# skipperro/selkies-gstreamer

Measured on AMD Instinct MI355X. Metric: encoded fps + glass-to-glass p50 ms at 1920x1080; concurrent 60fps sessions/node, higher is better.
Workload: dtype uint8 pixels / int32 integer transforms (bit-exact vs CPU reference); 1 GPU; model=H.264 Constrained Baseline CAVLC, striped stripes 64px, CRF 25, global_batch=8, seq_len=1, parallelism=session-parallel dp1 x 8 sessions/GPU, resolution=1920x1080, backend=hip, deblock=auto, me_full=True, upload_overlap=False, frames_in_flight=1, num_refs=1, numa_node_rank0=0

## Files before the change

csrc/kernels/h264_kernels.hip:

```cpp
#include "h264_gpu.h"
#include "../codec/color.h"
#include "../codec/h264_mb.h"
#include "../codec/h264_ep.h"

namespace sk {
namespace h264 {
namespace gpu {

__device__ __forceinline__ int lane_id() { return threadIdx.x & 63; }

__device__ __forceinline__ void wave_sync() {
    __builtin_amdgcn_fence(__ATOMIC_RELEASE, "wavefront");
    __builtin_amdgcn_wave_barrier();
    __builtin_amdgcn_fence(__ATOMIC_ACQUIRE, "wavefront");
}

__device__ __forceinline__ int wave_sum(int v) {
    v += __builtin_amdgcn_mov_dpp(v, 0xB1, 0xF, 0xF, false);
    v += __builtin_amdgcn_mov_dpp(v, 0x4E, 0xF, 0xF, false);
    v += __builtin_amdgcn_mov_dpp(v, 0x124, 0xF, 0xF, false);
    v += __builtin_amdgcn_mov_dpp(v, 0x128, 0xF, 0xF, false);
    return __builtin_amdgcn_readlane(v, 0) + __builtin_amdgcn_readlane(v, 16) +
           __builtin_amdgcn_readlane(v, 32) + __builtin_amdgcn_readlane(v, 48);
}
// ... 115 lines not shown
#ifdef SK_STAMPS
__device__ __forceinline__ void stamp(unsigned long long* dbg, int step, int point) {
    __builtin_amdgcn_sched_barrier(0);
    unsigned long long t = __builtin_amdgcn_s_memtime();
    __builtin_amdgcn_s_waitcnt(0xC07F);
    __builtin_amdgcn_sched_barrier(0);
    if (dbg && blockIdx.x == SK_STAMP_BLOCK && threadIdx.x == 0 && (unsigned)(step - SK_STAMP_STEP0) < 64u)
        dbg[(step - SK_STAMP_STEP0) * 16 + point] = t;
}
#define STAMP(step, pt) stamp(a.dbg, step, pt)
#define STAMP_S(dbg, step, pt) stamp(dbg, step, pt)
#else
#define STAMP(step, pt)
#define STAMP_S(dbg, step, pt)
#endif

struct AtomicBitWriter {
    uint32_t* buf;
    uint32_t pos;
    __device__ void put(uint32_t code, int len) {
        if (len <= 0) return;
        if (len < 32) code &= (1u << len) - 1u;
        uint32_t wi = pos >> 5, sh = pos & 31;
        if (sh + len <= 32) {
            atomicOr(&buf[wi], code << (32 - sh - len));
        } else {
            atomicOr(&buf[wi], code >> (sh + len - 32));
            atomicOr(&buf[wi + 1], code << (64 - sh - len));
        }
        pos += len;
    }
};

struct StageBitWriter {
    uint32_t* buf;
    uint32_t pos;
    uint32_t cap;
    bool ovf;
    __device__ void put(uint32_t code, int len) {
        if (len <= 0) return;
        if (pos + (uint32_t)len > cap) { ovf = true; pos += len; return; }
        if (len < 32) code &= (1u << len) - 1u;
        uint32_t wi = pos >> 5, sh = pos & 31;
        if (sh + len <= 32) {
            buf[wi] |= code << (32 - sh - len);
        } else {
            buf[wi] |= code >> (sh + len - 32);
            buf[wi + 1] |= code << (64 - sh - len);
        }
        pos += len;
    }
};

__device__ __forceinline__ uint32_t bgrx_px(const uint8_t* row, int x, int W) {
    return *reinterpret_cast<const uint32_t*>(row + 4 * sk_min(x, W - 1));
}

__global__ __launch_bounds__(256) void k_convert_damage(FrameArgs a) {
    __shared__ int mbd[16];
    const int t = threadIdx.x;
    if (t < 16) mbd[t] = 0;
    __syncthreads();
    const int item = t & 31, qr = t >> 5;
    const int mby = blockIdx.y, mbx0 = blockIdx.x * 16;
    const int x0 = mbx0 * 16 + item * 8;
    const int qy = mby * 8 + qr;
    bool diff = false;
    if (x0 < a.stride_y) {
        const int y0 = min(2 * qy, a.H - 1), y1 = min(2 * qy + 1, a.H - 1);
        const uint8_t* r0 = a.bgrx + (size_t)y0 * a.bgrx_stride;
        const uint8_t* r1 = a.bgrx + (size_t)y1 * a.bgrx_stride;
        uint32_t p0[8], p1[8];
        if (a.scaled) {
#pragma unroll
            for (int i = 0; i < 8; i++) {
                const int x = sk_min(x0 + i, a.W - 1);
                p0[i] = scale_fetch(a.bgrx, a.bgrx_stride, a.scale, x, y0);
                p1[i] = scale_fetch(a.bgrx, a.bgrx_stride, a.scale, x, y1);
            }
        } else if (x0 + 7 < a.W && (a.bgrx_stride & 15) == 0) {
            const uint4 a0 = *reinterpret_cast<const uint4*>(r0 + 4 * x0);
            const uint4 a1 = *reinterpret_cast<const uint4*>(r0 + 4 * x0 + 16);
            const uint4 b0 = *reinterpret_cast<const uint4*>(r1 + 4 * x0);
            const uint4 b1 = *reinterpret_cast<const uint4*>(r1 + 4 * x0 + 16);
            p0[0] = a0.x; p0[1] = a0.y; p0[2] = a0.z; p0[3] = a0.w;
            p0[4] = a1.x; p0[5] = a1.y; p0[6] = a1.z; p0[7] = a1.w;
            p1[0] = b0.x; p1[1] = b0.y; p1[2] = b0.z; p1[3] = b0.w;
            p1[4] = b1.x; p1[5] = b1.y; p1[6] = b1.z; p1[7] = b1.w;
        } else {
#pragma unroll
            for (int i = 0; i < 8; i++) {
                p0[i] = bgrx_px(r0, x0 + i, a.W);
                p1[i] = bgrx_px(r1, x0 + i, a.W);
            }
        }
        {
            const OverlayParams o0 = a.ov[0], o1 = a.ov[1];
            if (o0.on | o1.on) {
                const OverlayParams op[kOverlaySlots] = {o0, o1};
#pragma unroll
                for (int i = 0; i < 8; i++) {
                    const int x = sk_min(x0 + i, a.W - 1);
                    p0[i] = overlay_px(p0[i], x, y0, op, a.ov_img);
                    p1[i] = overlay_px(p1[i], x, y1, op, a.ov_img);
                }
            }
        }
        uint32_t ya[2] = {0, 0}, yb[2] = {0, 0}, cbw = 0, crw = 0;
#pragma unroll
        for (int q = 0; q < 4; q++) {
            uint8_t y[4], cb, cr;
            bgrx_quad_to_yuv((const uint8_t*)&p0[2 * q], (const uint8_t*)&p0[2 * q + 1], (const uint8_t*)&p1[2 * q],
                             (const uint8_t*)&p1[2 * q + 1], a.full_range, y, &cb, &cr);
            const int sh = 16 * (q & 1);
            ya[q >> 1] |= (uint32_t)(y[0] | (y[1] << 8)) << sh;
            yb[q >> 1] |= (uint32_t)(y[2] | (y[3] << 8)) << sh;
            cbw |= (uint32_t)cb << (8 * q);
            crw |= (uint32_t)cr << (8 * q);
        }
        const size_t oy = (size_t)(2 * qy) * a.stride_y + x0;
        const size_t oc = (size_t)qy * a.stride_c + x0 / 2;
        const uint2 pa = *reinterpret_cast<const uint2*>(a.prev.y + oy);
        const uint2 pb = *reinterpret_cast<const uint2*>(a.prev.y + oy + a.stride_y);
        const uint32_t pu = *reinterpret_cast<const uint32_t*>(a.prev.u + oc);
        const uint32_t pv = *reinterpret_cast<const uint32_t*>(a.prev.v + oc);
        diff = (pa.x != ya[0]) | (pa.y != ya[1]) | (pb.x != yb[0]) | (pb.y != yb[1]) | (pu != cbw) | (pv != crw);
        *reinterpret_cast<uint2*>(a.src.y + oy) = make_uint2(ya[0], ya[1]);
        *reinterpret_cast<uint2*>(a.src.y + oy + a.stride_y) = make_uint2(yb[0], yb[1]);
        *reinterpret_cast<uint32_t*>(a.src.u + oc) = cbw;
        *reinterpret_cast<uint32_t*>(a.src.v + oc) = crw;
    }
    if (diff || a.plan_ctl[1] == 0) mbd[item >> 1] = 1;
    __syncthreads();
    if (t < 16) {
        const int mbx = mbx0 + t;
        if (mbx < a.mb_w) a.mb_dirty[mby * a.mb_w + mbx] = (uint8_t)mbd[t];
    }
    if (__syncthreads_or(t < 16 && mbd[t] && mbx0 + t < a.mb_w) && t == 0)
        a.stripe_dirty[mby / a.rows_per_slice] = 1;
}

__global__ __launch_bounds__(256) void k_yuv_damage(FrameArgs a) {
    __shared__ int mbd[16];
    const int t = threadIdx.x;
    if (t < 16) mbd[t] = 0;
    __syncthreads();
    const int item = t & 31, qr = t >> 5;
    const int mby = blockIdx.y, mbx0 = blockIdx.x * 16;
    const int x0 = mbx0 * 16 + item * 8;
    const int qy = mby * 8 + qr;
    bool diff = false;
    if (x0 < a.stride_y) {
        const int W = a.W, H = a.H, cw = (W + 1) >> 1, ch = (H + 1) >> 1;
        const uint8_t* py = a.yuv;
        const uint8_t* pc = a.yuv + (size_t)W * H;
        const int y0 = min(2 * qy, H - 1), y1 = min(2 * qy + 1, H - 1), cy = min(qy, ch - 1);
        uint32_t ya[2] = {0, 0}, yb[2] = {0, 0}, cbw = 0, crw = 0;
#pragma unroll
        for (int i = 0; i < 8; i++) {
            const int x = min(x0 + i, W - 1);
            ya[i >> 2] |= (uint32_t)py[(size_t)y0 * W + x] << (8 * (i & 3));
            yb[i >> 2] |= (uint32_t)py[(size_t)y1 * W + x] << (8 * (i & 3));
        }
#pragma unroll
        for (int q = 0; q < 4; q++) {
            const int cx = min((x0 >> 1) + q, cw - 1);
            uint32_t u, v;
            if (a.yuv_fmt == 2) {
                const uint8_t* r = pc + (size_t)cy * (2 * cw) + 2 * cx;
                u = r[0];
                v = r[1];
            } else {
                u = pc[(size_t)cy * cw + cx];
                v = pc[(size_t)cw * ch + (size_t)cy * cw + cx];
            }
            cbw |= u << (8 * q);
            crw |= v << (8 * q);
        }
        const size_t oy = (size_t)(2 * qy) * a.stride_y + x0;
        const size_t oc = (size_t)qy * a.stride_c + x0 / 2;
        const uint2 pa = *reinterpret_cast<const uint2*>(a.prev.y + oy);
        const uint2 pb = *reinterpret_cast<const uint2*>(a.prev.y + oy + a.stride_y);
        const uint32_t pu = *reinterpret_cast<const uint32_t*>(a.prev.u + oc);
        const uint32_t pv = *reinterpret_cast<const uint32_t*>(a.prev.v + oc);
        diff = (pa.x != ya[0]) | (pa.y != ya[1]) | (pb.x != yb[0]) | (pb.y != yb[1]) | (pu != cbw) | (pv != crw);
        *reinterpret_cast<uint2*>(a.src.y + oy) = make_uint2(ya[0], ya[1]);
        *reinterpret_cast<uint2*>(a.src.y + oy + a.stride_y) = make_uint2(yb[0], yb[1]);
        *reinterpret_cast<uint32_t*>(a.src.u + oc) = cbw;
        *reinterpret_cast<uint32_t*>(a.src.v + oc) = crw;
    }
    if (diff || a.plan_ctl[1] == 0) mbd[item >> 1] = 1;
    __syncthreads();
    if (t < 16) {
        const int mbx = mbx0 + t;
        if (mbx < a.mb_w) a.mb_dirty[mby * a.mb_w + mbx] = (uint8_t)mbd[t];
    }
    if (__syncthreads_or(t < 16 && mbd[t] && mbx0 + t < a.mb_w) && t == 0)
        a.stripe_dirty[mby / a.rows_per_slice] = 1;
}

__device__ __forceinline__ uint32_t load_ref4(const uint8_t* row, int x, int stride) {
    if (x >= 0 && x + 3 <= stride - 1) {
        int xa = x & ~3, sh = x & 3;
        uint32_t w0 = *reinterpret_cast<const uint32_t*>(row + xa);
        if (sh == 0) return w0;
        uint32_t w1 = *reinterpret_cast<const uint32_t*>(row + xa + 4);
        return __builtin_amdgcn_alignbyte(w1, w0, sh);
    }
    uint32_t v = 0;
#pragma unroll
    for (int i = 0; i < 4; i++) v |= (uint32_t)row[sk_clip(x + i, 0, stride - 1)] << (8 * i);
    return v;
}

__device__ __forceinline__ uint32_t me_sad_lane(const FrameArgs& a, const uint8_t* refy, uint32_t sw, int mbx,
                                                int mby, int dx, int dy, int ylo, int yhi) {
    int l = lane_id();
    int row = l >> 2, col4 = (l & 3) * 4;
    int sy = sk_clip(mby * 16 + row + dy, ylo, yhi);
    uint32_t rw = load_ref4(refy + (size_t)sy * a.stride_y, mbx * 16 + col4 + dx, a.stride_y);
    return __builtin_amdgcn_sad_u8(sw, rw, 0u);
}

__device__ __forceinline__ int me_sad(const FrameArgs& a, const uint8_t* refy, uint32_t sw, int mbx,
                                      int mby, int dx, int dy, int ylo, int yhi) {
    return wave_sum((int)me_sad_lane(a, refy, sw, mbx, mby, dx, dy, ylo, yhi));
}

constexpr int kWin = 8;
constexpr int kWinWords = 10;
constexpr int kFsWinWords = kFsWin / 4 + 1;

struct MeWin {
    const uint32_t* w;
    int stride;
    int rad;
    int cx, cy;
    __device__ __forceinline__ bool has(int dx, int dy) const {
        return dx - cx >= -rad && dx - cx <= rad && dy - cy >= -rad && dy - cy <= rad;
    }
};

__device__ __forceinline__ uint32_t win_sad_lane(const MeWin& wn, uint32_t sw, int dx, int dy) {
    const int l = lane_id();
    const int row = l >> 2, col4 = (l & 3) * 4;
    const int bc = col4 + dx - wn.cx + wn.rad;
    const uint32_t* w = wn.w + (row + dy - wn.cy + wn.rad) * wn.stride + (bc >> 2);
    const int sh = bc & 3;
    const uint32_t rw = sh ? __builtin_amdgcn_alignbyte(w[1], w[0], sh) : w[0];
    return __builtin_amdgcn_sad_u8(sw, rw, 0u);
}
// ... 252 lines not shown
__global__ __launch_bounds__(256) void k_me(FrameArgs a) {
    __shared__ uint32_t win_s[4][kFsWin * kFsWinWords];
    __shared__ uint32_t blk_s[4][16 * kFsBlkWords];
    __shared__ __align__(16) int sq_s[4][kFsWin * kFsSqInts];
    static_assert(kFsWin * kFsWinWords >= 32 * kWinWords, "the small window lives in the wave's win_s region");
    const int w = threadIdx.x >> 6, l = lane_id();
    const int nmb = a.mb_w * a.mb_h;
    const int idx = xcd_remap(blockIdx.x, gridDim.x) * 4 + w;
    if (idx >= nmb) return;
    const int mbx = idx % a.mb_w, mby = idx / a.mb_w;
    const SliceTask t = a.tasks[mby / a.rows_per_slice];
    if (t.action != ACT_P && t.action != ACT_I) return;
    const uint32_t sw = *reinterpret_cast<const uint32_t*>(a.src.y + (size_t)(mby * 16 + (l >> 2)) * a.stride_y +
                                                           mbx * 16 + (l & 3) * 4);
    bool have_fs = false, big = false;
    int fsx = 0, fsy = 0;
    if (t.action == ACT_P && a.mb_dirty[idx]) {
        have_fs = true;
        const int ylo = t.pic_row0 * 16, yhi = (t.pic_row0 + t.pic_rows) * 16 - 1;
        const int R = a.me_range;
        const int px = sk_clip(a.mvfield[2 * idx], -R, R), py = sk_clip(a.mvfield[2 * idx + 1], -R, R);
        if (me_sad(a, a.ref.y, sw, mbx, mby, px, py, ylo, yhi) == 0) {
            fsx = px;
            fsy = py;
        } else {
            const uint64_t best = fs_search(a, win_s[w], blk_s[w], sq_s[w], mbx, mby, sw, ylo, yhi);
            fsx = __builtin_amdgcn_readfirstlane(fs_key_dx(best));
            fsy = __builtin_amdgcn_readfirstlane(fs_key_dy(best));
            big = true;
        }
        if (l == 0) {
            a.fs_mv[2 * idx] = (int16_t)fsx;
            a.fs_mv[2 * idx + 1] = (int16_t)fsy;
        }
    }
    me_search_mb(a, t, idx, mbx, mby, sw, have_fs, fsx, fsy, win_s[w], big);
}

__global__ __launch_bounds__(256) void k_plan(FrameArgs a) {
    const int ns = a.num_slices, tid = threadIdx.x;
    StripeState* st = a.plan_state;
    StripeState& pic = st[ns];
    if (a.plan_ctl[1] == 1) {
        if (a.fullframe) {
            bool idr = true;
            for (int s = tid; s < ns; s += 256) idr &= a.tasks[s].final_action == ACT_I && a.tasks[s].idr_on_intra;
            idr = __syncthreads_and(idr);
            if (tid == 0) commit_picture(pic, idr, a.plan_cfg.num_refs);
        } else {
            for (int s = tid; s < ns; s += 256) commit_stripe(st[s], a.tasks[s].final_action, a.plan_cfg.num_refs);
        }
    }
    __shared__ int hk[6];
    if (tid < 6) {
        hk[tid] = __hip_atomic_load(a.key_seq_host + tid, __ATOMIC_RELAXED, __HIP_MEMORY_SCOPE_SYSTEM);
        a.key_dev[tid] = hk[tid];
    }
    __syncthreads();
    const int kq = hk[0];
    const bool key = kq != a.plan_ctl[0];
    __syncthreads();
    if (key) {
        for (int s = tid; s < ns; s += 256) st[s].need_idr = true;
        if (tid == 0) pic.need_idr = true;
    }
    __syncthreads();
    PlanConfig pc = a.plan_cfg;
    const int qo = hk[1];
    const int po = hk[2];
    if (qo > 0) pc.qp = qo;
    if (po > 0) pc.paint_qp = po;
    {
        const int mode = hk[5] != a.rc->seq ? hk[3] : a.rc->mode;
        if (mode == RC_CBR) pc.use_paint_over = 0;
    }
    for (int s = tid; s < ns; s += 256) {
        st[s].subpel_prev = st[s].subpel_hits;
        st[s].subpel_hits = 0;
        const int r0 = s * a.rows_per_slice, nr = min(a.rows_per_slice, a.mb_h - r0);
        plan_stripe(pc, st[s], pic, a.stripe_dirty[s] != 0, r0, nr, a.mb_h, a.tasks[s]);
        a.stripe_dirty[s] = 0;
    }
    __syncthreads();
    if (tid == 0) {
        a.plan_ctl[0] = kq;
        a.plan_ctl[1] = 1;
    }
    if (tid < 4) a.frame_params_dev[tid] = a.frame_params_host[tid];
}

__global__ __launch_bounds__(256) void k_decide(FrameArgs a) {
    __shared__ long long red[2][4];
    const int s = blockIdx.x;
    SliceTask& t = a.tasks[s];
    const bool planned_p = t.action == ACT_P;
    const bool p = planned_p && t.allow_scenecut;
    long long sad = 0, dev = 0;
    if (planned_p || t.action == ACT_I) {
        const int first = t.first_row * a.mb_w, nmb = t.num_rows * a.mb_w;
        for (int i = threadIdx.x; i < nmb; i += 256) {
            const MeResult r = a.me[first + i];
            sad += r.sad;
            dev += r.intra_est;
        }
    }
    for (int o = 32; o > 0; o >>= 1) {
        sad += __shfl_down(sad, o);
        dev += __shfl_down(dev, o);
    }
    if (lane_id() == 0) {
        red[0][threadIdx.x >> 6] = sad;
        red[1][threadIdx.x >> 6] = dev;
    }
    __syncthreads();
    if (threadIdx.x == 0) {
        const long long ts = red[0][0] + red[0][1] + red[0][2] + red[0][3];
        const long long td = red[1][0] + red[1][1] + red[1][2] + red[1][3];
        t.final_action = (p && ts > td) ? ACT_I : t.action;
        a.rc_slice[2 * s] = ts;
        a.rc_slice[2 * s + 1] = td;
        a.tasks_host[s] = t;
    }
}

__device__ void rc_qp_serial(const FrameArgs& a) {
    RcState& rc = *a.rc;
    const int seq = a.key_dev[5];
    int plan_qp = a.plan_cfg.qp;
    const int qo = a.key_dev[1];
    if (qo > 0) plan_qp = qo;
    if (seq != rc.seq) {
        const int mode = a.key_dev[3];
        const int kbps = a.key_dev[4];
        const RcState old = rc;
        rc_init(rc, mode, plan_qp, kbps, (float)a.rc_fps, a.W * a.H, old.vbv_ms, old.codec);
        if (old.mode == mode)
            for (int k = 0; k < 2; k++) {
                rc.last_qp[k] = old.last_qp[k];
                rc.last_qpf[k] = old.last_qpf[k];
                rc.last_bits[k] = old.last_bits[k];
                rc.last_cplx[k] = old.last_cplx[k];
            }
        if (old.mode == mode) rc.cplx_ema = old.cplx_ema;
        rc.seq = seq;
    }
    rc.base_qp = plan_qp;
    rc_apply(rc, a.tasks, a.rc_slice, a.rc_slice + 1, a.num_slices, a.mb_w, plan_qp, 2);
}
__global__ __launch_bounds__(64) void k_rc_qp(FrameArgs a) {
    if (threadIdx.x == 0) rc_qp_serial(a);
    __syncthreads();
    for (int s = threadIdx.x; s < a.num_slices; s += 64) a.tasks_host[s].qp = a.tasks[s].qp;
}

__device__ __forceinline__ void rc_account_wave(const FrameArgs& a, const int* sizes, int n, int stride, int per_slice) {
    long long b = 0;
    for (int i = lane_id(); i < n; i += 64)
        if (!per_slice || i % per_slice < slice_nals(a, a.tasks[i / per_slice])) b += sizes[(size_t)i * stride];
    for (int o = 32; o > 0; o >>= 1) b += __shfl_down(b, o);
    if (lane_id() == 0) rc_account(*a.rc, 8 * b);
}

__global__ __launch_bounds__(64) void k_rc_account(FrameArgs a, const int* sizes, int n, int stride, int per_slice) {
    rc_account_wave(a, sizes, n, stride, per_slice);
}

__global__ __launch_bounds__(256) void k_rc_guard(FrameArgs a) {
    __shared__ long long part[4];
    const int s = blockIdx.x, tid = threadIdx.x;
    long long b = 0;
    for (int i = tid; i < a.num_slices; i += 256) {
        const int nn = slice_nals(a, a.tasks[i]);
        for (int j = 0; j < nn; j++) b += a.slice_info[4 * (i * a.nal_per_slice + j)];
    }
    for (int o = 32; o > 0; o >>= 1) b += __shfl_down(b, o);
    if ((tid & 63) == 0) part[tid >> 6] = b;
    __syncthreads();
    const long long bits = 8 * (part[0] + part[1] + part[2] + part[3]);
    const int step = rc_redo_step(*a.rc, bits);
    if (s == 0 && tid == 0) {
        const int applied = step ? rc_redo(*a.rc, a.tasks, a.num_slices, bits) : 0;
        *a.rc_redo = applied ? 1 : 0;
        if (applied)
            for (int i = 0; i < a.num_slices; i++) a.tasks_host[i].qp = a.tasks[i].qp;
    }
    if (!step || a.tasks[s].final_action == ACT_NONE) return;
    const int nn = slice_nals(a, a.tasks[s]);
    for (int j = 0; j < nn; j++) {
        uint32_t* rbsp = nal_rbsp(a, s, j);
        const int words = (a.slice_info[4 * (s * a.nal_per_slice + j)] + 3) / 4 + 1;
        for (int i = tid; i < words; i += 256) rbsp[i] = 0u;
    }
}

__global__ __launch_bounds__(256) void k_rc_guard_sizes(FrameArgs a, const int* sizes, int n, int* redo, int chained) {
    __shared__ long long part[4];
    if (chained && *redo == 0) return;
    const int tid = threadIdx.x;
    long long b = 0;
    for (int i = tid; i < n; i += 256) b += sizes[i];
    for (int o = 32; o > 0; o >>= 1) b += __shfl_down(b, o);
    if ((tid & 63) == 0) part[tid >> 6] = b;
    __syncthreads();
    if (tid != 0) return;
    const long long bits = 8 * (part[0] + part[1] + part[2] + part[3]);
    const int applied = rc_redo_step(*a.rc, bits) ? rc_redo(*a.rc, a.tasks, a.num_slices, bits) : 0;
    *redo = applied ? 1 : 0;
    if (applied)
        for (int i = 0; i < a.num_slices; i++) a.tasks_host[i].qp = a.tasks[i].qp;
}

struct MbScratch {
    int16_t coef[kCoefPerMb];
    int dcy[16];
    int dcc[8];
    int blk_stat[32];
    int misc[8];
    uint8_t nnz[24];
    uint8_t pad[8];
    int cdcp[8];
    uint8_t nb[64];
    uint8_t nbtr[4];
    uint8_t ref13[32];
    uint8_t ry[256];
};

__device__ __forceinline__ void lds_hadamard4x4(int* x) {
    const int l = lane_id();
    if (l < 4) {
        int a = x[l * 4 + 0], b = x[l * 4 + 1], c = x[l * 4 + 2], d = x[l * 4 + 3];
        int s01 = a + b, d01 = a - b, s23 = c + d, d23 = c - d;
        x[l * 4 + 0] = s01 + s23;
        x[l * 4 + 1] = s01 - s23;
        x[l * 4 + 2] = d01 - d23;
        x[l * 4 + 3] = d01 + d23;
    }
    wave_sync();
    if (l < 4) {
        int a = x[l], b = x[4 + l], c = x[8 + l], d = x[12 + l];
        int s01 = a + b, d01 = a - b, s23 = c + d, d23 = c - d;
        x[l] = s01 + s23;
        x[4 + l] = s01 - s23;
        x[8 + l] = d01 - d23;
        x[12 + l] = d01 + d23;
    }
// ... 1421 lines not shown
    } else if (l <= 18) {
        if (cbp_c) { act = true; bc = coef + kCoefChromaDC + (l - 17) * 4; maxn = 4; nc = -1; }
    } else if (l <= 26) {
        if (cbp_c == 2) {
            int k = l - 19, c = k >> 2, bb = k & 3;
            act = true; bc = coef + kCoefChromaAC + (c * 4 + bb) * 16 + 1; maxn = 15;
            nc = chroma_nc(mb, nb, c, bb);
        }
    }
    int nbits = 0;
    uint32_t* stage = stage_all + (l < 27 ? l : 0) * kCavlcStageWords;
    StageBitWriter sw{stage, 0, kCavlcStageWords * 32, false};
    if (act) {
        cavlc_block(sw, bc, maxn, nc, T);
        nbits = (int)sw.pos;
    }
    int incl = wave_incl_scan(nbits);
    int off = hdr_bits + incl - nbits;
    if (act) {
        if (!sw.ovf) {
            const uint32_t sh = (uint32_t)off & 31;
            uint32_t wi = (uint32_t)off >> 5;
            for (int k = 0; k < (nbits + 31) >> 5; k++, wi++) {
                const uint32_t v = stage[k];
                atomicOr(&bits[wi], v >> sh);
                const uint32_t lo = sh ? v << (32 - sh) : 0u;
                if (lo) atomicOr(&bits[wi + 1], lo);
            }
        } else {
            AtomicBitWriter w{bits, (uint32_t)off};
            cavlc_block(w, bc, maxn, nc, T);
        }
    }
    int total = hdr_bits + __shfl(incl, 63);
    wave_sync();
    int nwords = (total + 31) >> 5;
    uint32_t* dst = a.mb_bits + (size_t)idx * (kMbSlotBytes / 4);
    for (int i = l; i < nwords; i += 64) dst[i] = bits[i];
    if (l == 0) a.mb_nbits[idx] = total;
}

constexpr int kTile = 4096;

__global__ __launch_bounds__(256) void k_slice_scan(FrameArgs a) {
    if (a.gate && *a.gate == 0) return;
    __shared__ uint32_t hdr[32];
    __shared__ int wave_tot[5];
    __shared__ int sh_misc[4];
    const int nal = blockIdx.x, s = nal / a.nal_per_slice, j = nal % a.nal_per_slice, tid = threadIdx.x;
    const SliceTask task = a.tasks[s];
    const int fin = task.final_action;
    int* info = a.slice_info + 4 * nal;
    const int nn = slice_nals(a, task);
    if (j >= nn) {
        if (tid == 0) {
            info[0] = 0;
            info[1] = 0;
            if (j == 0) a.host_size[s] = 0;
        }
        return;
    }
    const int snmb = task.num_rows * a.mb_w;
    const int k0 = nn > 1 ? j * kIntraSubMbs : 0;
    const int nmb = nn > 1 ? sk_min(snmb, k0 + kIntraSubMbs) - k0 : snmb;
    const int first = task.first_row * a.mb_w + k0;
    uint32_t* rbsp = nal_rbsp(a, s, j);
    const bool intra = fin == ACT_I;
    const bool idr = intra && task.idr_on_intra;
    if (tid < 32) hdr[tid] = 0;
    if (tid == 0) sh_misc[1] = -1;
    __syncthreads();
    if (tid == 0) {
        AtomicBitWriter w{hdr, 0};
        SliceHeaderParams h;
        h.first_mb = (a.fullframe ? task.first_row * a.mb_w : 0) + k0;
        h.slice_type = intra ? 2 : 0;
        h.idr = idr;
        h.frame_num = idr ? 0 : task.frame_num;
        h.idr_pic_id = task.idr_pic_id;
        h.slice_qp = task.qp;
        h.deblock = slice_deblock(a.deblock, task);
        h.num_refs = intra ? 1 : task.num_refs;
        write_slice_header(w, h);
        if (fin == ACT_SKIPALL) put_ue(w, (uint32_t)nmb);
        sh_misc[0] = (int)w.pos;
    }
    const int per = (nmb + 255) / 256;
    const int m0 = sk_min(nmb, tid * per), m1 = sk_min(nmb, m0 + per);
    int local = 0, last_coded = -1;
    if (fin != ACT_SKIPALL)
        for (int m = m0; m < m1; m++) {
            const int nb = a.mb_nbits[first + m];
            local += nb;
            if (nb > 0) last_coded = m;
        }
    if (last_coded >= 0) atomicMax(&sh_misc[1], last_coded);
    int total;
    const int excl = block_excl_scan<4>(local, wave_tot, &total);
    const int hb = sh_misc[0];
    if (fin != ACT_SKIPALL) {
        int off = hb + excl;
        for (int m = m0; m < m1; m++) {
            a.mb_off[first + m] = off;
            off += a.mb_nbits[first + m];
        }
    }
// ... 517 lines not shown
                uint8_t* p0 = dst + rowoff + xb * mbbytes;
                *reinterpret_cast<uint2*>(p0) = make_uint2(q.x, q.y);
                *reinterpret_cast<uint2*>(p0 + half2) = chroma ? make_uint2(q.x, q.y) : make_uint2(q.z, q.w);
            }
        }
        lds_barrier();
    }
}

void launch_convert_damage(const FrameArgs& a, hipStream_t s) {
    dim3 grid((a.mb_w + 15) / 16, a.mb_h);
    if (a.yuv_fmt) hipLaunchKernelGGL(k_yuv_damage, grid, dim3(256), 0, s, a);
    else hipLaunchKernelGGL(k_convert_damage, grid, dim3(256), 0, s, a);
}

void launch_frontend(const FrameArgs& a, hipStream_t s) {
    int nmb = a.mb_w * a.mb_h;
    hipLaunchKernelGGL(k_plan, dim3(1), dim3(256), 0, s, a);
    if (a.me_full) hipLaunchKernelGGL(k_me, dim3((nmb + 3) / 4), dim3(256), 0, s, a);
    else hipLaunchKernelGGL(k_motion_search, dim3(nmb), dim3(64), 0, s, a);
    hipLaunchKernelGGL(k_decide, dim3(a.num_slices), dim3(256), 0, s, a);
    hipLaunchKernelGGL(k_rc_qp, dim3(1), dim3(64), 0, s, a);
    if (a.subpel) hipLaunchKernelGGL(k_subpel, dim3((nmb + 3) / 4), dim3(256), 0, s, a);
}

void launch_rc_guard_sizes(const FrameArgs& a, const int* sizes, int n, int* redo, bool chained, hipStream_t s) {
    hipLaunchKernelGGL(k_rc_guard_sizes, dim3(1), dim3(256), 0, s, a, sizes, n, redo, chained ? 1 : 0);
}

void launch_rc_account(const FrameArgs& a, const int* sizes, int n, int stride, int per_slice, hipStream_t s) {
    hipLaunchKernelGGL(k_rc_account, dim3(1), dim3(64), 0, s, a, sizes, n, stride, per_slice);
}

static void launch_code(const FrameArgs& a, hipStream_t s) {
    int nmb = a.mb_w * a.mb_h;
    hipLaunchKernelGGL(k_code_inter, dim3((nmb + 3) / 4), dim3(256), 0, s, a);
    hipLaunchKernelGGL(k_intra_prep, dim3((nmb + 3) / 4), dim3(256), 0, s, a);
    if (a.rows_per_slice <= 4)
        hipLaunchKernelGGL(k_code_intra<4>, dim3(a.num_slices), dim3(64 * 5), 0, s, a);
    else
        hipLaunchKernelGGL(k_code_intra<kMaxRows - 1>, dim3(a.num_slices), dim3(64 * kMaxRows), 0, s, a);
    if (a.nal_per_slice > 1)
        hipLaunchKernelGGL(k_code_intra_sub, dim3((a.num_slices * a.nal_per_slice + 3) / 4), dim3(256), 0, s, a);
    hipLaunchKernelGGL(k_cavlc, dim3((nmb + 3) / 4), dim3(256), 0, s, a);
    hipLaunchKernelGGL(k_slice_scan, dim3(a.num_slices * a.nal_per_slice), dim3(256), 0, s, a);
}

void launch_encode(const FrameArgs& a, hipStream_t s, bool guard) {
    int nmb = a.mb_w * a.mb_h;
    launch_frontend(a, s);
    if (a.aq_strength > 0) hipLaunchKernelGGL(k_aq, dim3((nmb + 3) / 4), dim3(256), 0, s, a);
    launch_code(a, s);
    if (guard && a.rc_redo) {
        hipLaunchKernelGGL(k_rc_guard, dim3(a.num_slices), dim3(256), 0, s, a);
        FrameArgs b = a;
        b.gate = a.rc_redo;
        launch_code(b, s);
    }
    hipLaunchKernelGGL(k_mb_concat, dim3((nmb + 3) / 4), dim3(256), 0, s, a);
    const dim3 tiles(a.max_tiles, a.num_slices);
    hipLaunchKernelGGL(k_ep_count, tiles, dim3(256), 0, s, a);
    hipLaunchKernelGGL(k_ep_write, tiles, dim3(256), 0, s, a);
}

void launch_commit(const FrameArgs& a, hipStream_t s) {
    hipLaunchKernelGGL(k_commit, dim3((a.mb_w + 15) / 16, a.mb_h), dim3(256), 0, s, a);
    if (a.deblock) {
        const int nmb = a.mb_w * a.mb_h;
        hipLaunchKernelGGL(k_deblock_prep, dim3((nmb + 3) / 4), dim3(256), 0, s, a);
        hipLaunchKernelGGL(k_deblock_edges, dim3((nmb + 255) / 256), dim3(256), 0, s, a);
        if (a.rows_per_slice <= 4)
            hipLaunchKernelGGL(k_deblock<4>, dim3(a.num_slices), dim3(64 * a.rows_per_slice), 0, s, a);
        else
            hipLaunchKernelGGL(k_deblock<kMaxRows>, dim3(a.num_slices), dim3(64 * a.rows_per_slice), 0, s, a);
    }
}

}
}
}
```

csrc/runtime/h264_hip.cpp:

```cpp
#include "encoder_iface.h"
#include "trace.h"
#include "../kernels/h264_gpu.h"
#include "../kernels/hevc_gpu.h"
#include "../kernels/av1_gpu.h"
#include "../codec/av1_encoder.h"
#include "../kernels/runtime_kernels.h"
#include "../codec/hevc_encoder.h"
#include <hip/hip_runtime.h>
#include <atomic>
#include <chrono>
#include <map>
#include <mutex>
#include <stdexcept>
#include <string.h>
#include <string>
#include <thread>
#include <vector>
#include <atomic>

namespace sk {
namespace {

#define HIPCHECK(x)                                                                     \
    do {                                                                                \
// ... 167 lines not shown
            }
            up_valid_[0] = up_valid_[1] = false;
            invalidate_graphs();
            args_.bgrx_stride = stride;
        }
        if (inflight() >= 2) {
            set_last_error("upload(): two frames in flight; finish() the oldest first");
            return -1;
        }
        const int q = launched_ & 1;
        if (staged_) up_valid_[0] = up_valid_[1] = false;
        hipStream_t cs = stream_;
        if (copy_stream_) cs = copy_stream_;
        else if (inflight() && upload_mode_ != 0) cs = upload_mode_ == 2 ? device_copy_stream(device_) : upload_stream();
        if (ext_wait_) {
            HIPCHECK(hipStreamWaitEvent(cs, ev_ext_, 0));
            ext_wait_ = false;
        }
        HIPCHECK(hipEventRecord(ev_[3 * q], cs));
        upload_copy(q, bgrx, stride, in_bytes, cs);
        if (cs != stream_) HIPCHECK(hipEventRecord(ev_copy_[q], cs));
        staged_on_main_ = cs == stream_;
        staged_ = true;
        staged_frame_ = frame_id;
        return 0;
    }

    int wait_stream(void* stream) override {
        HIPCHECK(hipSetDevice(device_));
        if (!ev_ext_) HIPCHECK(hipEventCreateWithFlags(&ev_ext_, hipEventDisableTiming));
        HIPCHECK(hipEventRecord(ev_ext_, (hipStream_t)stream));
        ext_wait_ = true;
        return 0;
    }

    int launch() override {
        if (!staged_ || inflight() >= 2) {
            set_last_error("launch() needs one uploaded frame and at most one frame in flight");
            return -1;
        }
        trace::Range frame_range("h264.launch");
        HIPCHECK(hipSetDevice(device_));
        const int p = launched_ & 1;
        parity_ = p;
        if ((cfg_.rc_mode == RC_CBR) != graph_guard_) {
            HIPCHECK(hipStreamSynchronize(stream_));
            invalidate_graphs();
            graph_guard_ = cfg_.rc_mode == RC_CBR;
        }
        set_parity_args(args_.bgrx_stride);
        h_frame_params_[p][0] = staged_frame_;
        for (int i = 0; i < 6; i++) h_key_snap_[p][i] = __atomic_load_n(&h_key_seq_[i], __ATOMIC_SEQ_CST);
        frame_of_[p] = staged_frame_;
        memcpy(ov_params_host_[p], ov_pending_, sizeof(ov_pending_));
        if (!staged_on_main_) HIPCHECK(hipStreamWaitEvent(stream_, ev_copy_[p], 0));
        HIPCHECK(hipEventRecord(ev_[3 * p + 1], stream_));
        run_graph(graph_exec_[p], 0);
        HIPCHECK(hipEventRecord(ev_[3 * p + 2], stream_));
        run_graph(post_exec_[p], 1);
        staged_ = false;
        launched_++;
        parity_ = launched_ & 1;
        return 0;
    }

    int finish() override {
        if (inflight() <= 0) {
            set_last_error("finish() without a launched frame");
            return -1;
        }
        const int p = finished_ & 1;
        {
            trace::Range r("h264.wait");
            HIPCHECK(hipEventSynchronize(ev_[3 * p + 2]));
        }
        {
            trace::Range r("h264.packets");
            packets_.clear();
            build_packets(p, frame_of_[p]);
        }
        finished_++;
        float t0 = 0, t1 = 0;
        hipEventElapsedTime(&t0, ev_[3 * p], ev_[3 * p + 1]);
        hipEventElapsedTime(&t1, ev_[3 * p + 1], ev_[3 * p + 2]);
        stage_ms_[0] = t0;
        stage_ms_[1] = t1;
        return (int)packets_.size();
    }

    int64_t state_bytes() override { return (int64_t)h264::state_bytes(g_); }

    void xfer(void* dst, const void* src, size_t n, bool to_caller, int on_device) {
        const hipMemcpyKind k = on_device ? hipMemcpyDeviceToDevice
                                          : (to_caller ? hipMemcpyDeviceToHost : hipMemcpyHostToDevice);
        HIPCHECK(hipMemcpyAsync(dst, src, n, k, stream_));
    }

    int export_state(void* dst, int on_device) override {
        HIPCHECK(hipSetDevice(device_));
        HIPCHECK(hipStreamSynchronize(stream_));
        const int ns = g_.num_slices;
        int ctl[4];
        std::vector<StripeState> st(ns + 1);
        std::vector<SliceTask> tasks(ns);
        copy_now(ctl, args_.plan_ctl, sizeof(ctl));
        copy_now(st.data(), args_.plan_state, sizeof(StripeState) * (ns + 1));
        copy_now(tasks.data(), args_.tasks, sizeof(SliceTask) * ns);
// ... 152 lines not shown
            return n;
        } else return -1;
        if (dst && cap >= n) HIPCHECK(hipMemcpyAsync(dst, p, (size_t)n, hipMemcpyDeviceToHost, stream_));
        HIPCHECK(hipStreamSynchronize(stream_));
        return n;
    }

   private:
    template <class T>
    T* dmalloc(size_t count, bool zero = true) {
        void* p = nullptr;
        HIPCHECK(hipMalloc(&p, count * sizeof(T)));
        if (zero) HIPCHECK(hipMemsetAsync(p, 0, count * sizeof(T), stream_));
        dev_allocs_.push_back(p);
        return (T*)p;
    }
    template <class T>
    T* hmalloc(size_t count, unsigned flags = hipHostMallocDefault) {
        void* p = nullptr;
        HIPCHECK(hipHostMalloc(&p, count * sizeof(T), flags));
        memset(p, 0, count * sizeof(T));
        host_allocs_.push_back(p);
        return (T*)p;
    }

    gpu::Planes make_planes() {
        size_t ny = (size_t)g_.stride_y * g_.plane_h_y, nc = (size_t)g_.stride_c * g_.plane_h_c;
        gpu::Planes p;
        p.y = dmalloc<uint8_t>(ny);
        p.u = dmalloc<uint8_t>(nc);
        p.v = dmalloc<uint8_t>(nc);
        return p;
    }

    void alloc() {
        const int nmb = g_.num_mbs(), ns = g_.num_slices;
        planes_src_[0] = make_planes();
        planes_src_[1] = make_planes();
        gpu::FrameArgs& a = args_;
        memset(&a, 0, sizeof(a));
        a.W = g_.W; a.H = g_.H; a.mb_w = g_.mb_w; a.mb_h = g_.mb_h;
        a.stride_y = g_.stride_y; a.stride_c = g_.stride_c;
        a.num_slices = ns; a.rows_per_slice = g_.rows_per_slice; a.fullframe = cfg_.fullframe;
        a.full_range = cfg_.full_range; a.me_range = cfg_.me_range; a.me_iters = cfg_.me_iters;
        a.deblock = cfg_.codec == 0 ? cfg_.deblock : 0;
        a.me_full = cfg_.me_full;
        a.aq_strength = cfg_.codec == 1 ? 0 : cfg_.aq_strength;
        a.subpel = cfg_.codec == 2 ? 0 : cfg_.subpel;
        a.intra4x4 = cfg_.codec == 1 ? 0 : cfg_.intra4x4;
        a.aq = dmalloc<int8_t>(nmb);
        for (int k = 0; k < kOverlaySlots; k++) {
            ov_img_dev_[k] = dmalloc<uint8_t>((size_t)kOverlayMaxDim * kOverlayMaxDim * 4);
            a.ov_img[k] = ov_img_dev_[k];
            ov_params_host_[k] = hmalloc<OverlayParams>(kOverlaySlots);
        }
        ov_params_dev_ = dmalloc<OverlayParams>(kOverlaySlots);
        a.ov = ov_params_dev_;
        memset(ov_pending_, 0, sizeof(ov_pending_));
        a.num_refs = cfg_.num_refs > 1 ? 2 : 1;
        a.scaled = (cfg_.src_width > 0 && cfg_.src_width != cfg_.width) ||
                   (cfg_.src_height > 0 && cfg_.src_height != cfg_.height);
        if (a.scaled)
            a.scale = scale_params(cfg_.src_width > 0 ? cfg_.src_width : cfg_.width,
                                   cfg_.src_height > 0 ? cfg_.src_height : cfg_.height, cfg_.width, cfg_.height);
        a.ref = make_planes();
        a.ref1 = make_planes();
        a.rec = make_planes();
        a.mb_dirty = dmalloc<uint8_t>(nmb);
        void* dd = nullptr;
        a.stripe_dirty = dmalloc<int>(ns);
        a.plan_ctl = dmalloc<int>(4);
        a.plan_cfg = plan_config(cfg_);
        {
            std::vector<StripeState> init(ns + 1);
            a.plan_state = dmalloc<StripeState>(ns + 1);
            HIPCHECK(hipMemcpyAsync(a.plan_state, init.data(), sizeof(StripeState) * (ns + 1),
                                    hipMemcpyHostToDevice, stream_));
            HIPCHECK(hipStreamSynchronize(stream_));
        }
        h_key_seq_ = hmalloc<int>(16, hipHostMallocCoherent);
        for (int p = 0; p < 2; p++) {
            h_key_snap_[p] = hmalloc<int>(8, hipHostMallocCoherent);
            HIPCHECK(hipHostGetDevicePointer(&dd, h_key_snap_[p], 0));
            key_snap_dev_[p] = (const int*)dd;
        }
        a.key_seq_host = key_snap_dev_[0];
        a.key_dev = dmalloc<int>(8);
        a.tasks = dmalloc<SliceTask>(ns);
        a.me = dmalloc<MeResult>(nmb);
        a.mvfield = dmalloc<int16_t>(2 * nmb);
        a.fs_mv = dmalloc<int16_t>(2 * nmb);
        {
            RcState rc;
            rc_init(rc, cfg_.rc_mode, cfg_.qp, cfg_.bitrate_kbps, cfg_.fps, cfg_.width * cfg_.height, cfg_.vbv_ms, cfg_.codec);
            a.rc = dmalloc<RcState>(1);
            copy_now(a.rc, &rc, sizeof(rc));
            a.rc_slice = dmalloc<long long>(2 * (size_t)ns);
            a.rc_redo = dmalloc<int>(1);
            a.gate = nullptr;
            a.rc_fps = cfg_.fps;
            h_key_seq_[3] = cfg_.rc_mode;
            h_key_seq_[4] = cfg_.bitrate_kbps;
        }
        a.db = dmalloc<DbInfo>(nmb);
        a.dbe = dmalloc<uint4>((size_t)3 * nmb);
        a.mbs = dmalloc<MbInfo>(nmb);
        a.coefs = dmalloc<int16_t>((size_t)nmb * kCoefPerMb);
        a.mb_bits = dmalloc<uint32_t>((size_t)nmb * (gpu::kMbSlotBytes / 4));
// ... 29 lines not shown
            ps.resize(ns);
            for (int s = 0; s < ns; s++) build_parameter_sets(g_.W, g_.slice_pix_h(s), cfg_.full_range, cfg_.fps, ps[s], cfg_.num_refs);
        }
        param_sets_ = ps;
        a.param_set_stride = 256;
        std::vector<uint8_t> flat((size_t)ns * 256, 0);
        std::vector<int> lens(ns, 0);
        for (int s = 0; s < ns; s++) {
            const std::vector<uint8_t>& v = ps[cfg_.fullframe ? 0 : s];
            if (v.size() > 256) throw std::runtime_error("parameter sets too large");
            memcpy(&flat[(size_t)s * 256], v.data(), v.size());
            lens[s] = (int)v.size();
        }
        uint8_t* dps = dmalloc<uint8_t>(flat.size());
        HIPCHECK(hipMemcpyAsync(dps, flat.data(), flat.size(), hipMemcpyHostToDevice, stream_));
        HIPCHECK(hipStreamSynchronize(stream_));
        int* dlen = dmalloc<int>(ns);
        HIPCHECK(hipMemcpyAsync(dlen, lens.data(), sizeof(int) * ns, hipMemcpyHostToDevice, stream_));
        HIPCHECK(hipStreamSynchronize(stream_));
        a.param_sets = dps;
        a.param_set_len = dlen;
        CavlcTables* ct = dmalloc<CavlcTables>(1);
        HIPCHECK(hipMemcpyAsync(ct, &host_cavlc_tables(), sizeof(CavlcTables), hipMemcpyHostToDevice, stream_));
        HIPCHECK(hipStreamSynchronize(stream_));
        a.cavlc_tabs = ct;
        d_frame_params_ = dmalloc<int>(4);
        if (getenv("SK_STAMPS")) a.dbg = dmalloc<unsigned long long>(64 * 16 + 256);
        a.frame_params_dev = d_frame_params_;
        for (int p = 0; p < 2; p++) {
            h_tasks_[p] = hmalloc<SliceTask>(ns, hipHostMallocCoherent);
            HIPCHECK(hipHostGetDevicePointer(&dd, h_tasks_[p], 0));
            tasks_host_dev_[p] = (SliceTask*)dd;
            h_frame_params_[p] = hmalloc<int>(4, hipHostMallocCoherent);
            HIPCHECK(hipHostGetDevicePointer(&dd, h_frame_params_[p], 0));
            frame_params_dev_host_[p] = (const int*)dd;
        }
    }

    void set_parity_args(int stride) {
        args_.yuv = yuv_dev_[parity_];
        args_.yuv_fmt = yuv_mode_;
        args_.bgrx = bgrx_dev_[parity_];
        args_.bgrx_stride = stride;
        args_.src = planes_src_[parity_];
        args_.prev = planes_src_[parity_ ^ 1];
        args_.host_out = host_out_dev_[parity_];
        args_.host_size = host_size_dev_[parity_];
        args_.tasks_host = tasks_host_dev_[parity_];
        args_.frame_params_host = frame_params_dev_host_[parity_];
        args_.key_seq_host = key_snap_dev_[parity_];
    }

    void invalidate_graphs() {
        for (auto* set : {graph_exec_, post_exec_})
            for (int i = 0; i < 2; i++)
                if (set[i]) { hipGraphExecDestroy(set[i]); set[i] = nullptr; }
    }

    void enqueue(int part) {
        if (part == 0) {
            HIPCHECK(hipMemcpyAsync(ov_params_dev_, ov_params_host_[parity_], sizeof(OverlayParams) * kOverlaySlots,
                                    hipMemcpyHostToDevice, stream_));
            gpu::launch_convert_damage(args_, stream_);
            if (cfg_.codec == 2) {
                gpu::launch_frontend(args_, stream_);
                av1::gpu::Av1Args aa = aargs_;
                aa.f = args_;
                aa.frame_host = av1_frame_dev_[parity_];
                aa.out_host = av1_out_dev_[parity_];
                aa.out_size_host = av1_size_dev_[parity_];
                av1::gpu::launch_backend(aa, stream_, graph_guard_ ? args_.rc_redo : nullptr);
                gpu::launch_rc_account(args_, aa.tile_size, av1_geo_.tile_cols * av1_geo_.tile_rows, 1, 0, stream_);
            } else if (cfg_.codec == 1) {
                gpu::launch_frontend(args_, stream_);
                hevc::gpu::HevcArgs ha = hargs_;
                ha.f = args_;
                ha.out_host = hevc_out_dev_[parity_];
                ha.out_size = hevc_size_dev_[parity_];
                ha.out_dev = hevc_fallback_[parity_];
                hevc::gpu::launch_backend(ha, stream_, graph_guard_ ? args_.rc_redo : nullptr);
                gpu::launch_rc_account(args_, ha.sub_size, ha.ch * ha.seg_k, 1, 0, stream_);
            } else {
                gpu::launch_encode(args_, stream_, graph_guard_);
            }
        } else {
            gpu::launch_commit(args_, stream_);
        }
    }

    void run_graph(hipGraphExec_t& gx, int part) {
        if (!use_graphs_) {
            enqueue(part);
            return;
        }
        if (!gx) {
            hipGraph_t graph;
            HIPCHECK(hipStreamBeginCapture(stream_, hipStreamCaptureModeRelaxed));
            enqueue(part);
            HIPCHECK(hipStreamEndCapture(stream_, &graph));
            HIPCHECK(hipGraphInstantiate(&gx, graph, nullptr, nullptr, 0));
            hipGraphDestroy(graph);
        }
        HIPCHECK(hipGraphLaunch(gx, stream_));
    }

    void alloc_hevc() {
        const int n = g_.num_mbs(), ns = g_.num_slices;
        hevc::Geo geo;
        geo.init(g_);
        hevc::gpu::HevcArgs& h = hargs_;
        memset(&h, 0, sizeof(h));
        h.cw = geo.ctb_w;
        h.ch = geo.ctb_h;
        h.rps = geo.rows_per_slice;
        if (g_.rows_per_slice & 1) throw std::runtime_error("HEVC: stripes must be whole CTB rows");
// ... 224 lines not shown
    Geometry g_;
    Controller ctl_;
    int device_;
    hevc::gpu::HevcArgs hargs_;
    av1::gpu::Av1Args aargs_;
    av1::Av1Geo av1_geo_;
    int av1_level_ = 8;
    uint8_t* av1_out_[2] = {nullptr, nullptr};
    uint8_t* av1_out_dev_[2] = {nullptr, nullptr};
    int* av1_size_[2] = {nullptr, nullptr};
    int* av1_size_dev_[2] = {nullptr, nullptr};
    int* av1_frame_[2] = {nullptr, nullptr};
    int* av1_frame_dev_[2] = {nullptr, nullptr};
    uint8_t* hevc_out_[2] = {nullptr, nullptr};
    uint8_t* hevc_out_dev_[2] = {nullptr, nullptr};
    int* hevc_size_[2] = {nullptr, nullptr};
    int* hevc_size_dev_[2] = {nullptr, nullptr};
    uint8_t* hevc_fallback_[2] = {nullptr, nullptr};
    std::vector<uint8_t> hevc_params_;
    hipStream_t stream_ = nullptr;
    hipEvent_t ev_[6];
    gpu::FrameArgs args_;
    gpu::Planes planes_src_[2];
    int parity_ = 0;
    uint8_t* bgrx_dev_[2] = {nullptr, nullptr};
    hipEvent_t ev_copy_[2];
    bool staged_ = false, staged_on_main_ = true;
    int launched_ = 0, finished_ = 0;
    int inflight() const { return launched_ - finished_; }
    uint16_t frame_of_[2] = {0, 0};
    uint16_t staged_frame_ = 0;
    size_t bgrx_cap_ = 0;
    bool up_valid_[2] = {false, false};
    bool up_next_known_ = false, up_prev_known_ = false;
    std::vector<int> up_next_, up_prev_;
    std::atomic<long long> up_rows_copied_{0}, up_rows_total_{0};
    uint8_t* host_out_[2] = {nullptr, nullptr};
    uint8_t* host_out_dev_[2] = {nullptr, nullptr};
    int* host_size_dev_[2] = {nullptr, nullptr};
    SliceTask* tasks_host_dev_[2] = {nullptr, nullptr};
    const int* frame_params_dev_host_[2] = {nullptr, nullptr};
    int* h_key_seq_ = nullptr;
    SliceTask* h_tasks_[2] = {nullptr, nullptr};
    int* h_out_size_[2] = {nullptr, nullptr};
    int* h_frame_params_[2] = {nullptr, nullptr};
    int* h_key_snap_[2] = {nullptr, nullptr};
    const int* key_snap_dev_[2] = {nullptr, nullptr};
    int* d_frame_params_ = nullptr;
    std::vector<std::vector<uint8_t>> param_sets_;
    std::vector<void*> dev_allocs_, host_allocs_;
    hipGraphExec_t graph_exec_[2] = {nullptr, nullptr};
    uint8_t* ov_img_dev_[kOverlaySlots] = {};
    OverlayParams* ov_params_dev_ = nullptr;
    OverlayParams* ov_params_host_[2] = {};
    OverlayParams ov_pending_[kOverlaySlots];
    uint8_t* ov_stage_ = nullptr;
    hipGraphExec_t post_exec_[2] = {nullptr, nullptr};
    bool use_graphs_ = getenv("SK_NO_GRAPHS") == nullptr;
    void copy_now(void* dst, const void* src, size_t n) {
        HIPCHECK(hipMemcpyAsync(dst, src, n, hipMemcpyDefault, stream_));
        HIPCHECK(hipStreamSynchronize(stream_));
    }
    bool graph_guard_ = false;
    uint8_t* yuv_dev_[2] = {nullptr, nullptr};
    int yuv_mode_ = 0;
    hipEvent_t ev_ext_ = nullptr;
    bool ext_wait_ = false;
    hipStream_t copy_stream_ = nullptr;
    hipStream_t up_stream_ = nullptr;
    int upload_mode_ = getenv("SK_UPLOAD_MODE") ? atoi(getenv("SK_UPLOAD_MODE")) : 2;
    hipStream_t upload_stream() {
        if (!up_stream_) HIPCHECK(hipStreamCreateWithFlags(&up_stream_, hipStreamNonBlocking));
        return up_stream_;
    }

    static hipStream_t device_copy_stream(int device) {
        static std::mutex mu;
        static std::map<int, hipStream_t> streams;
        std::lock_guard<std::mutex> lk(mu);
        auto it = streams.find(device);
        if (it != streams.end()) return it->second;
        hipStream_t s = nullptr;
        HIPCHECK(hipStreamCreateWithFlags(&s, hipStreamNonBlocking));
        streams[device] = s;
        return s;
    }
    float stage_ms_[4] = {0, 0, 0, 0};
};

}

void warm_copy_engines(int device) {
    static std::mutex mu;
    static std::map<int, bool> done;
    std::lock_guard<std::mutex> lk(mu);
    if (done[device]) return;
    done[device] = true;
    const char* env = getenv("SK_COPY_WARMUP");
    if (env && atoi(env) == 0) return;
    const int kThreads = 8, kRounds = 60, kKernels = 12;
    const size_t bytes = (size_t)8 << 20;
    uint8_t* host = nullptr;
    if (hipHostMalloc((void**)&host, bytes, hipHostMallocDefault) != hipSuccess) return;
    for (size_t i = 0; i < bytes; i += 4096) host[i] = 0;
    std::vector<std::thread> th;
    for (int t = 0; t < kThreads; t++)
        th.emplace_back([=] {
// ... 27 lines not shown
```

Before: 5627 frames/s (1920x1080 H.264, all sessions, all GPUs).

## Trim per-frame serial work: hoist host-word loads, LDS rate control, lazy overlay upload

Several small serial costs on the per-frame critical path are reduced. The system-scope loads of key and frame-param words move into the first damage kernel, so k_plan reads device copies. k_rc_qp stages tasks, sums and RC state in LDS before the single-thread serial rate-control pass. k_rc_guard shrinks to one block, and the clearing of stale bitstream moves into the redo code kernel. The overlay parameter upload leaves the captured graph and is sent from the host only when the parameters change, which risks overlay updates going stale if the resend logic is wrong.

```diff
diff --git a/csrc/kernels/h264_kernels.hip b/csrc/kernels/h264_kernels.hip
--- a/csrc/kernels/h264_kernels.hip
+++ b/csrc/kernels/h264_kernels.hip
@@ -191,6 +191,19 @@
     }
 };
 
+__device__ __forceinline__ int host_words_load(const FrameArgs& a) {
+    const int tid = threadIdx.x;
+    if (blockIdx.x != 0 || blockIdx.y != 0 || tid >= 10) return 0;
+    return __hip_atomic_load(tid < 6 ? a.key_seq_host + tid : a.frame_params_host + (tid - 6), __ATOMIC_RELAXED,
+                             __HIP_MEMORY_SCOPE_SYSTEM);
+}
+__device__ __forceinline__ void host_words_store(const FrameArgs& a, int v) {
+    const int tid = threadIdx.x;
+    if (blockIdx.x != 0 || blockIdx.y != 0 || tid >= 10) return;
+    if (tid < 6) a.key_dev[tid] = v;
+    else a.frame_params_dev[tid - 6] = v;
+}
+
 __device__ __forceinline__ uint32_t bgrx_px(const uint8_t* row, int x, int W) {
     return *reinterpret_cast<const uint32_t*>(row + 4 * sk_min(x, W - 1));
 }
@@ -198,6 +211,7 @@
 __global__ __launch_bounds__(256) void k_convert_damage(FrameArgs a) {
     __shared__ int mbd[16];
     const int t = threadIdx.x;
+    const int host_words = host_words_load(a);
     if (t < 16) mbd[t] = 0;
     __syncthreads();
     const int item = t & 31, qr = t >> 5;
@@ -277,11 +291,13 @@
     }
     if (__syncthreads_or(t < 16 && mbd[t] && mbx0 + t < a.mb_w) && t == 0)
         a.stripe_dirty[mby / a.rows_per_slice] = 1;
+    host_words_store(a, host_words);
 }
 
 __global__ __launch_bounds__(256) void k_yuv_damage(FrameArgs a) {
     __shared__ int mbd[16];
     const int t = threadIdx.x;
+    const int host_words = host_words_load(a);
     if (t < 16) mbd[t] = 0;
     __syncthreads();
     const int item = t & 31, qr = t >> 5;
@@ -336,6 +352,7 @@
     }
     if (__syncthreads_or(t < 16 && mbd[t] && mbx0 + t < a.mb_w) && t == 0)
         a.stripe_dirty[mby / a.rows_per_slice] = 1;
+    host_words_store(a, host_words);
 }
 
 __device__ __forceinline__ uint32_t load_ref4(const uint8_t* row, int x, int stride) {
@@ -694,10 +711,7 @@
         }
     }
     __shared__ int hk[6];
-    if (tid < 6) {
-        hk[tid] = __hip_atomic_load(a.key_seq_host + tid, __ATOMIC_RELAXED, __HIP_MEMORY_SCOPE_SYSTEM);
-        a.key_dev[tid] = hk[tid];
-    }
+    if (tid < 6) hk[tid] = a.key_dev[tid];
     __syncthreads();
     const int kq = hk[0];
     const bool key = kq != a.plan_ctl[0];
@@ -728,7 +742,6 @@
         a.plan_ctl[0] = kq;
         a.plan_ctl[1] = 1;
     }
-    if (tid < 4) a.frame_params_dev[tid] = a.frame_params_host[tid];
 }
 
 __global__ __launch_bounds__(256) void k_decide(FrameArgs a) {
@@ -765,15 +778,14 @@
     }
 }
 
-__device__ void rc_qp_serial(const FrameArgs& a) {
-    RcState& rc = *a.rc;
-    const int seq = a.key_dev[5];
+__device__ void rc_qp_serial(const FrameArgs& a, const int* key, RcState& rc, SliceTask* tasks, const long long* sums) {
+    const int seq = key[5];
     int plan_qp = a.plan_cfg.qp;
-    const int qo = a.key_dev[1];
+    const int qo = key[1];
     if (qo > 0) plan_qp = qo;
     if (seq != rc.seq) {
-        const int mode = a.key_dev[3];
-        const int kbps = a.key_dev[4];
+        const int mode = key[3];
+        const int kbps = key[4];
         const RcState old = rc;
         rc_init(rc, mode, plan_qp, kbps, (float)a.rc_fps, a.W * a.H, old.vbv_ms, old.codec);
         if (old.mode == mode)
@@ -787,12 +799,35 @@
         rc.seq = seq;
     }
     rc.base_qp = plan_qp;
-    rc_apply(rc, a.tasks, a.rc_slice, a.rc_slice + 1, a.num_slices, a.mb_w, plan_qp, 2);
-}
+    rc_apply(rc, tasks, sums, sums + 1, a.num_slices, a.mb_w, plan_qp, 2);
+}
+constexpr int kRcLdsSlices = 128;
 __global__ __launch_bounds__(64) void k_rc_qp(FrameArgs a) {
-    if (threadIdx.x == 0) rc_qp_serial(a);
+    __shared__ long long sums_l[2 * kRcLdsSlices];
+    __shared__ SliceTask tasks_l[kRcLdsSlices];
+    __shared__ RcState rc_l;
+    __shared__ int key_l[6];
+    static_assert(sizeof(RcState) % 4 == 0 && sizeof(SliceTask) % 4 == 0, "dword copies");
+    const int ns = a.num_slices, l = threadIdx.x;
+    const bool in_lds = ns <= kRcLdsSlices;
+    if (in_lds) {
+        for (int i = l; i < ns * (int)(sizeof(SliceTask) / 4); i += 64)
+            reinterpret_cast<uint32_t*>(tasks_l)[i] = reinterpret_cast<const uint32_t*>(a.tasks)[i];
+        for (int i = l; i < 2 * ns; i += 64) sums_l[i] = a.rc_slice[i];
+        if (l < (int)(sizeof(RcState) / 4)) reinterpret_cast<uint32_t*>(&rc_l)[l] = reinterpret_cast<const uint32_t*>(a.rc)[l];
+        if (l < 6) key_l[l] = a.key_dev[l];
+    }
     __syncthreads();
-    for (int s = threadIdx.x; s < a.num_slices; s += 64) a.tasks_host[s].qp = a.tasks[s].qp;
+    if (l == 0) {
+        if (in_lds) rc_qp_serial(a, key_l, rc_l, tasks_l, sums_l);
+        else rc_qp_serial(a, a.key_dev, *a.rc, a.tasks, a.rc_slice);
+    }
+    __syncthreads();
+    if (in_lds) {
+        if (l < (int)(sizeof(RcState) / 4)) reinterpret_cast<uint32_t*>(a.rc)[l] = reinterpret_cast<const uint32_t*>(&rc_l)[l];
+        for (int s = l; s < ns; s += 64) a.tasks[s].qp = tasks_l[s].qp;
+    }
+    for (int s = l; s < ns; s += 64) a.tasks_host[s].qp = in_lds ? tasks_l[s].qp : a.tasks[s].qp;
 }
 
 __device__ __forceinline__ void rc_account_wave(const FrameArgs& a, const int* sizes, int n, int stride, int per_slice) {
@@ -809,7 +844,7 @@
 
 __global__ __launch_bounds__(256) void k_rc_guard(FrameArgs a) {
     __shared__ long long part[4];
-    const int s = blockIdx.x, tid = threadIdx.x;
+    const int tid = threadIdx.x;
     long long b = 0;
     for (int i = tid; i < a.num_slices; i += 256) {
         const int nn = slice_nals(a, a.tasks[i]);
@@ -818,21 +853,12 @@
     for (int o = 32; o > 0; o >>= 1) b += __shfl_down(b, o);
     if ((tid & 63) == 0) part[tid >> 6] = b;
     __syncthreads();
+    if (tid != 0) return;
     const long long bits = 8 * (part[0] + part[1] + part[2] + part[3]);
-    const int step = rc_redo_step(*a.rc, bits);
-    if (s == 0 && tid == 0) {
-        const int applied = step ? rc_redo(*a.rc, a.tasks, a.num_slices, bits) : 0;
-        *a.rc_redo = applied ? 1 : 0;
-        if (applied)
-            for (int i = 0; i < a.num_slices; i++) a.tasks_host[i].qp = a.tasks[i].qp;
-    }
-    if (!step || a.tasks[s].final_action == ACT_NONE) return;
-    const int nn = slice_nals(a, a.tasks[s]);
-    for (int j = 0; j < nn; j++) {
-        uint32_t* rbsp = nal_rbsp(a, s, j);
-        const int words = (a.slice_info[4 * (s * a.nal_per_slice + j)] + 3) / 4 + 1;
-        for (int i = tid; i < words; i += 256) rbsp[i] = 0u;
-    }
+    const int applied = rc_redo_step(*a.rc, bits) ? rc_redo(*a.rc, a.tasks, a.num_slices, bits) : 0;
+    *a.rc_redo = applied ? 1 : 0;
+    if (applied)
+        for (int i = 0; i < a.num_slices; i++) a.tasks_host[i].qp = a.tasks[i].qp;
 }
 
 __global__ __launch_bounds__(256) void k_rc_guard_sizes(FrameArgs a, const int* sizes, int n, int* redo, int chained) {
@@ -2360,6 +2386,12 @@
     const int fin = task.final_action;
     int* info = a.slice_info + 4 * nal;
     const int nn = slice_nals(a, task);
+    if (a.gate && info[0] > 0) {
+        uint32_t* old = nal_rbsp(a, s, j);
+        const int words = (info[0] + 3) / 4 + 1;
+        for (int i = tid; i < words; i += 256) old[i] = 0u;
+        __syncthreads();
+    }
     if (j >= nn) {
         if (tid == 0) {
             info[0] = 0;
@@ -2983,7 +3015,7 @@
     if (a.aq_strength > 0) hipLaunchKernelGGL(k_aq, dim3((nmb + 3) / 4), dim3(256), 0, s, a);
     launch_code(a, s);
     if (guard && a.rc_redo) {
-        hipLaunchKernelGGL(k_rc_guard, dim3(a.num_slices), dim3(256), 0, s, a);
+        hipLaunchKernelGGL(k_rc_guard, dim3(1), dim3(256), 0, s, a);
         FrameArgs b = a;
         b.gate = a.rc_redo;
         launch_code(b, s);
diff --git a/csrc/runtime/h264_hip.cpp b/csrc/runtime/h264_hip.cpp
--- a/csrc/runtime/h264_hip.cpp
+++ b/csrc/runtime/h264_hip.cpp
@@ -243,7 +243,14 @@
         h_frame_params_[p][0] = staged_frame_;
         for (int i = 0; i < 6; i++) h_key_snap_[p][i] = __atomic_load_n(&h_key_seq_[i], __ATOMIC_SEQ_CST);
         frame_of_[p] = staged_frame_;
-        memcpy(ov_params_host_[p], ov_pending_, sizeof(ov_pending_));
+        if (ov_resend_ || memcmp(ov_sent_, ov_pending_, sizeof(ov_pending_)) != 0) {
+            memcpy(ov_params_host_[ov_slot_], ov_pending_, sizeof(ov_pending_));
+            HIPCHECK(hipMemcpyAsync(ov_params_dev_, ov_params_host_[ov_slot_], sizeof(ov_pending_),
+                                    hipMemcpyHostToDevice, stream_));
+            memcpy(ov_sent_, ov_pending_, sizeof(ov_pending_));
+            ov_slot_ = (ov_slot_ + 1) % kOvStage;
+            ov_resend_ = false;
+        }
         if (!staged_on_main_) HIPCHECK(hipStreamWaitEvent(stream_, ev_copy_[p], 0));
         HIPCHECK(hipEventRecord(ev_[3 * p + 1], stream_));
         run_graph(graph_exec_[p], 0);
@@ -502,8 +509,8 @@
         for (int k = 0; k < kOverlaySlots; k++) {
             ov_img_dev_[k] = dmalloc<uint8_t>((size_t)kOverlayMaxDim * kOverlayMaxDim * 4);
             a.ov_img[k] = ov_img_dev_[k];
-            ov_params_host_[k] = hmalloc<OverlayParams>(kOverlaySlots);
-        }
+        }
+        for (auto& h : ov_params_host_) h = hmalloc<OverlayParams>(kOverlaySlots);
         ov_params_dev_ = dmalloc<OverlayParams>(kOverlaySlots);
         a.ov = ov_params_dev_;
         memset(ov_pending_, 0, sizeof(ov_pending_));
@@ -639,6 +646,7 @@
     }
 
     void invalidate_graphs() {
+        ov_resend_ = true;
         for (auto* set : {graph_exec_, post_exec_})
             for (int i = 0; i < 2; i++)
                 if (set[i]) { hipGraphExecDestroy(set[i]); set[i] = nullptr; }
@@ -646,8 +654,6 @@
 
     void enqueue(int part) {
         if (part == 0) {
-            HIPCHECK(hipMemcpyAsync(ov_params_dev_, ov_params_host_[parity_], sizeof(OverlayParams) * kOverlaySlots,
-                                    hipMemcpyHostToDevice, stream_));
             gpu::launch_convert_damage(args_, stream_);
             if (cfg_.codec == 2) {
                 gpu::launch_frontend(args_, stream_);
@@ -978,7 +984,11 @@
     hipGraphExec_t graph_exec_[2] = {nullptr, nullptr};
     uint8_t* ov_img_dev_[kOverlaySlots] = {};
     OverlayParams* ov_params_dev_ = nullptr;
-    OverlayParams* ov_params_host_[2] = {};
+    static constexpr int kOvStage = 2;
+    OverlayParams* ov_params_host_[kOvStage] = {};
+    OverlayParams ov_sent_[kOverlaySlots] = {};
+    int ov_slot_ = 0;
+    bool ov_resend_ = true;
     OverlayParams ov_pending_[kOverlaySlots];
     uint8_t* ov_stage_ = nullptr;
     hipGraphExec_t post_exec_[2] = {nullptr, nullptr};
```

New measurement: 5731 frames/s (1920x1080 H.264, all sessions, all GPUs) (median of 6 runs). 1.8% higher.
